# pandegroup/deepchem

Measured on AMD Instinct MI355X. Metric: molecules/sec fwd+bwd GraphConvModel, higher is better.
Workload: dtype f32; 1 GPU; Tox21-like synthetic molecules (18.2 atoms/mol, E/N 2.08), 12 binary tasks, GraphConvModel [64,64]/dense 128, BatchNorm on, fwd+bwd+Adam per step; grad_mode=full, gemm_mode=fast (split-bf16 x3 products on v_mfma_f32_32x32x16_bf16, fp32-accurate), parallelism=dp1 (molecules sharded by rank, one flat all-reduce per step)

## Files before the change

deepchem_amd/csrc/bwd_fused.hip:

```cpp
#include <atomic>
#include <type_traits>

#include "common.h"
#include "split_bf16.h"

namespace gcmi {

constexpr int kFRows = 64;
constexpr int kFMaxSeg = 16;

struct FusedTable {
  int32_t n_seg;
  int32_t seg_begin[kFMaxSeg];
  int32_t seg_end[kFMaxSeg];
  int32_t tile_start[kFMaxSeg + 1];
  int64_t w_off[2][kFMaxSeg];
  int64_t db_off[kFMaxSeg];
};

struct FusedArgs {
  const float* dy;
  int32_t lddy;
  const float* x;
  int32_t ldx;
  const float* coef;
  const int32_t* membership;
  const float* g2;
  int32_t ldg2;
  const int32_t* arg;
  const float* in[2];
  int32_t ldin[2];
  int32_t k_in;
  const float* w;
  float* dw;
  float* db;
  float* dout[2];
  int32_t lddout[2];
  double* psums;
  unsigned long long* diag;
};

template <int NG, int KT, int NOPS, bool TRANS, bool RD, bool DGRAD, bool HB = false, bool GB = false, bool IB = HB>
__global__ void __launch_bounds__(DGRAD ? 512 : 256) __attribute__((amdgpu_waves_per_eu(2)))
fused_bwd_kernel(FusedTable st, int n_tiles, FusedArgs a, int rev) {
  static_assert(!GB || HB, "bf16 gradient streams come with bf16 activations");
  static_assert(IB || !HB, "bf16 activations include the block's inputs");
  static_assert(IB == HB || !DGRAD, "In alone as bf16: the weight-gradient-only form");
  constexpr int NT = DGRAD ? 512 : 256;
  constexpr int NJ = NG / 32;
  constexpr int KP = KT * 32;
  constexpr int GP = NG + 4;
  constexpr int IP = KP + 4;
  constexpr int WP = NG + 8;
  constexpr size_t kWBytes = !DGRAD ? 0 : sizeof(unsigned short) * (size_t)NOPS * 3 * KP * WP;
  constexpr int QPR = NG / 4;
  constexpr int RPP = NT / QPR;
  constexpr int GPASS = kFRows / RPP;
  constexpr int IQ = KP / 4;
  constexpr int IPASS = kFRows * IQ / NT;
  constexpr int STEPS = kFRows / 16;
  constexpr bool INTERLEAVE = !RD;
  constexpr int OT = NOPS * KT;
  constexpr int TPW = OT / 2;
  constexpr int OP = OT * 32 + 8;
  constexpr int OQ = OT * 8;
  constexpr int OPASS = DGRAD ? kFRows * OQ / NT : 1;
  static_assert(NOPS * NJ == 4, "four weight-gradient waves: one (operand, column group) each");
  static_assert(!DGRAD || (OT % 2 == 0), "input-gradient tiles split over two waves per row block");
  static_assert(kFRows * IQ % NT == 0, "In tile loads divide evenly");
  extern __shared__ __attribute__((aligned(16))) unsigned char lds_raw[];
  float* Gs = reinterpret_cast<float*>(lds_raw);
  float* Ins = Gs + kFRows * GP;
  unsigned short* Wimg = reinterpret_cast<unsigned short*>(Ins + NOPS * kFRows * IP);
  float* Outs = reinterpret_cast<float*>(reinterpret_cast<unsigned char*>(Wimg) + kWBytes);
  __shared__ int t_begin_s[kFMaxSeg], t_end_s[kFMaxSeg], t_tile_s[kFMaxSeg + 1];
  __shared__ long long t_w_s[2][kFMaxSeg], t_db_s[kFMaxSeg];
  __shared__ __attribute__((aligned(16))) float coef_s[3 * NG];
  __shared__ double stat_s[2][DGRAD ? KP : 1];

  const int tid = threadIdx.x;
  const int wave = __builtin_amdgcn_readfirstlane(tid >> 6);
  const int lane = tid & 63;
  const int half = lane >> 5;
  const int l31 = lane & 31;
  const bool is_dgrad = DGRAD && wave < 4;
  const int wq = wave & 3;
  const int wo = wq / NJ, wj = wq % NJ;
  const int rb = wq & 1, cg = wq >> 1;

  if (tid <= kFMaxSeg) {
    t_tile_s[tid] = pick_n(st.tile_start, tid);
    if (tid < kFMaxSeg) {
      t_begin_s[tid] = pick_n(st.seg_begin, tid);
      t_end_s[tid] = pick_n(st.seg_end, tid);
      t_w_s[0][tid] = pick_n(st.w_off[0], tid);
      t_w_s[1][tid] = pick_n(st.w_off[1], tid);
      t_db_s[tid] = pick_n(st.db_off, tid);
    }
  }
  const int n_seg = st.n_seg;

  const int b = rev ? (int)gridDim.x - 1 - (int)blockIdx.x : (int)blockIdx.x;
  const int t_begin = (int)((int64_t)b * n_tiles / gridDim.x);
  const int t_end = (int)((int64_t)(b + 1) * n_tiles / gridDim.x);
  const int my_tiles = t_end - t_begin;
  auto tile_at = [&](int i) { return rev ? t_end - 1 - i : t_begin + i; };

  const int gq = tid % QPR;
  const int gr = tid / QPR;
  for (int c = tid; c < 3 * NG; c += NT) coef_s[c] = a.coef != nullptr ? a.coef[c] : (c < NG ? 1.f : 0.f);
  if constexpr (DGRAD)
    for (int c = tid; c < 2 * KP; c += NT) stat_s[c / KP][c % KP] = 0.0;

  __syncthreads();

  struct Cursor { int seg, t0, t1, r0, r1; } cur;
  auto cur_load = [&]() {
    cur.t0 = __builtin_amdgcn_readfirstlane(t_tile_s[cur.seg]);
    cur.t1 = __builtin_amdgcn_readfirstlane(t_tile_s[cur.seg + 1]);
    cur.r0 = __builtin_amdgcn_readfirstlane(t_begin_s[cur.seg]);
    cur.r1 = __builtin_amdgcn_readfirstlane(t_end_s[cur.seg]);
  };
  {
    const int first = tile_at(0);
    int sg = 0;
    for (int k = 1; k < n_seg; ++k) sg += first >= t_tile_s[k] ? 1 : 0;
    cur.seg = __builtin_amdgcn_readfirstlane(sg);
    cur_load();
  }
  auto tile_info = [&](int tile, int& seg, int& row0, int& valid) {
    while (tile >= cur.t1) { ++cur.seg; cur_load(); }
    while (tile < cur.t0) { --cur.seg; cur_load(); }
    seg = cur.seg;
    row0 = cur.r0 + (tile - cur.t0) * kFRows;
    const int left = cur.r1 - row0;
    valid = left < kFRows ? left : kFRows;
  };

  using ActV = typename std::conditional<HB, uint2, float4>::type;
  auto load_act = [](const float* base, unsigned elem) -> ActV {
    if constexpr (HB) return *reinterpret_cast<const uint2*>(reinterpret_cast<const bf16_t*>(base) + elem);
    else return *reinterpret_cast<const float4*>(base + elem);
  };
  auto act4 = [](const ActV& v) -> float4 {
    if constexpr (HB) return widen4(v);
    else return v;
  };
  using InV = typename std::conditional<IB, uint2, float4>::type;
  auto load_in = [](const float* base, unsigned elem) -> InV {
    if constexpr (IB) return *reinterpret_cast<const uint2*>(reinterpret_cast<const bf16_t*>(base) + elem);
    else return *reinterpret_cast<const float4*>(base + elem);
  };
  auto in4 = [](const InV& v) -> float4 {
    if constexpr (IB) return widen4(v);
    else return v;
  };
  using DyV = typename std::conditional<GB && !RD, uint2, float4>::type;
  DyV pdy[GPASS];
  float4 pgm[RD ? GPASS : 1];
  ActV px[GPASS];
  InV pin[NOPS][IPASS];
  int4 parg[RD ? GPASS : 1];
  int mem1[RD ? GPASS : 1];
  auto clampr = [](int r, int valid) { return r < valid ? r : valid - 1; };
  auto load_mem = [&](int row0, int valid, int (&mem)[RD ? GPASS : 1]) {
    if constexpr (RD) {
#pragma unroll
      for (int p = 0; p < GPASS; ++p) mem[p] = a.membership[(unsigned)(row0 + clampr(gr + p * RPP, valid))];
    }
  };
  auto load_src = [&](int row0, int valid) {
#pragma unroll
    for (int p = 0; p < GPASS; ++p) {
      const unsigned r = (unsigned)(row0 + clampr(gr + p * RPP, valid));
      px[p] = load_act(a.x, r * (unsigned)a.ldx + 4u * gq);
      if constexpr (RD) {
        const unsigned m = (unsigned)mem1[p];
        pdy[p] = *reinterpret_cast<const float4*>(a.g2 + (m * (unsigned)a.ldg2 + 4u * gq));
        pgm[p] = *reinterpret_cast<const float4*>(a.g2 + (m * (unsigned)a.ldg2 + NG + 4u * gq));
        parg[p] = *reinterpret_cast<const int4*>(a.arg + (m * (unsigned)NG + 4u * gq));
      } else {
        if constexpr (GB) pdy[p] = *reinterpret_cast<const uint2*>(reinterpret_cast<const bf16_t*>(a.dy) + (r * (unsigned)a.lddy + 4u * gq));
        else pdy[p] = *reinterpret_cast<const float4*>(a.dy + (r * (unsigned)a.lddy + 4u * gq));
      }
    }
#pragma unroll
    for (int o = 0; o < NOPS; ++o) {
#pragma unroll
      for (int p = 0; p < IPASS; ++p) {
        const int slot = tid + p * NT;
        const int r = slot / IQ, q = slot - r * IQ;
        const int ld = a.ldin[o];
        const int qc = 4 * q + 4 <= ld ? 4 * q : 0;
        pin[o][p] = load_in(a.in[o], (unsigned)(row0 + clampr(r, valid)) * (unsigned)ld + qc);
      }
    }
  };

  constexpr int NACC = (DGRAD && TPW > KT) ? TPW : KT;
  f32x16 accs[NACC];
#pragma unroll
  for (int t = 0; t < NACC; ++t)
#pragma unroll
    for (int i = 0; i < 16; ++i) accs[t][i] = 0.f;
  float bsum = 0.f;
  auto flush_w = [&](int seg) {
    const int64_t woff = t_w_s[NOPS == 2 ? wo : 0][seg];
    if (woff >= 0) {
      int64_t woff_lane = woff + (TRANS ? (int64_t)(wj * 32 + 4 * half) * a.k_in + l31
                                        : (int64_t)(4 * half) * NG + wj * 32 + l31);
      asm volatile("" : "+v"(woff_lane));
      float* wp = a.dw + woff_lane;
#pragma unroll
      for (int t = 0; t < KT; ++t) {
#pragma unroll
        for (int reg = 0; reg < 16; ++reg) {
          const int r8 = (reg & 3) + 8 * (reg >> 2);
          if constexpr (TRANS) {
            if (t * 32 + l31 < a.k_in) atomicAdd(wp + (int64_t)r8 * a.k_in + t * 32, accs[t][reg]);
          } else {
            if (t * 32 + r8 + 4 * half < a.k_in) atomicAdd(wp + (t * 32 + r8) * NG, accs[t][reg]);
          }
        }
      }
    }
#pragma unroll
    for (int t = 0; t < KT; ++t)
#pragma unroll
      for (int i = 0; i < 16; ++i) accs[t][i] = 0.f;
    if (wo == 0) {
      const int64_t boff = t_db_s[seg];
      const float s = bsum + __shfl_xor(bsum, 32);
      if (half == 0 && a.db != nullptr && boff >= 0) atomicAdd(a.db + boff + wj * 32 + l31, s);
    }
    bsum = 0.f;
  };

  static_assert(!DGRAD || NT % IQ == 0, "a thread keeps its column piece over the passes");
  float ps1[4] = {0.f, 0.f, 0.f, 0.f}, ps2[4] = {0.f, 0.f, 0.f, 0.f};
  auto flush_psums = [&]() {
    if constexpr (DGRAD) {
      const int q = tid % IQ;
      if (4 * q < a.k_in) {
#pragma unroll
        for (int i = 0; i < 4; ++i) {
          atomicAdd(&stat_s[0][4 * q + i], (double)ps1[i]);
          atomicAdd(&stat_s[1][4 * q + i], (double)ps2[i]);
          ps1[i] = ps2[i] = 0.f;
        }
      }
    }
  };
  auto store_out = [&](int prow0, int pvalid, int pseg) {
    if constexpr (DGRAD) {
      static_assert(OQ == NOPS * IQ, "one input-gradient row piece per In row piece");
      const float deg = (float)pseg;
#pragma unroll
      for (int o = 0; o < NOPS; ++o) {
        float* dst = o == 1 ? a.dout[1] : a.dout[0];
        const int ldd = o == 1 ? a.lddout[1] : a.lddout[0];
#pragma unroll
        for (int p = 0; p < IPASS; ++p) {
          const int slot = tid + p * NT;
          const int r = slot / IQ, q = slot - r * IQ;
          if (r < pvalid && 4 * q < a.k_in) {
            float4 v = *reinterpret_cast<const float4*>(Outs + r * OP + o * KP + 4 * q);
            if constexpr (GB) {
              const uint2 h = narrow4(v.x, v.y, v.z, v.w);
              *reinterpret_cast<uint2*>(reinterpret_cast<bf16_t*>(dst) + ((unsigned)(prow0 + r) * (unsigned)ldd + 4u * q)) = h;
              v = widen4(h);
            } else {
              *reinterpret_cast<float4*>(dst + ((unsigned)(prow0 + r) * (unsigned)ldd + 4u * q)) = v;
            }
            if (a.psums != nullptr) {
              const float4 in = *reinterpret_cast<const float4*>(Ins + (o * kFRows + r) * IP + 4 * q);
              const float wgt = (NOPS == 2 && o == 0) ? deg : 1.f;
              ps1[0] = fmaf(wgt, v.x, ps1[0]); ps1[1] = fmaf(wgt, v.y, ps1[1]);
              ps1[2] = fmaf(wgt, v.z, ps1[2]); ps1[3] = fmaf(wgt, v.w, ps1[3]);
              ps2[0] = fmaf(v.x, in.x, ps2[0]); ps2[1] = fmaf(v.y, in.y, ps2[1]);
              ps2[2] = fmaf(v.z, in.z, ps2[2]); ps2[3] = fmaf(v.w, in.w, ps2[3]);
            }
          }
        }
      }
    }
  };

  int seg, row0, valid;
  tile_info(tile_at(0), seg, row0, valid);
  int nseg = seg, nrow0 = row0, nvalid = valid;
  if (my_tiles > 1) tile_info(tile_at(1), nseg, nrow0, nvalid);
  load_mem(row0, valid, mem1);
  load_src(row0, valid);
  load_mem(nrow0, nvalid, mem1);
  int cur_seg = -1;
  int prow0 = row0, pvalid = 0, pseg = 0;

  const bool stamp = a.diag != nullptr && blockIdx.x == 0 && lane == 0 && (wave == 0 || wave == NT / 64 - 1);
  unsigned long long d_a = 0, d_w1 = 0, d_b = 0, d_w2 = 0, t0 = 0, t1 = 0;
  for (int i = 0; i < my_tiles; ++i) {
    if (stamp) t0 = wall_clock64();
    if (seg != cur_seg) {
      if (cur_seg >= 0 && !is_dgrad) flush_w(cur_seg);
      cur_seg = seg;
      if constexpr (DGRAD) {
        constexpr int NE = NOPS * KP * NG;
        for (int e = tid; e < NE; e += NT) {
          int o, ko, c;
          if constexpr (TRANS) {
            o = 0;
            c = e / KP;
            ko = e - c * KP;
          } else {
            o = e / (KP * NG);
            const int r = e - o * (KP * NG);
            ko = r / NG;
            c = r - ko * NG;
          }
          const int64_t woff = t_w_s[NOPS == 2 ? (o & 1) : 0][seg];
          float v = 0.f;
          if (woff >= 0 && ko < a.k_in)
            v = TRANS ? a.w[woff + (int64_t)c * a.k_in + ko] : a.w[woff + (int64_t)ko * NG + c];
          unsigned p1, p2, p3;
          split3(v, p1, p2, p3);
          unsigned short* dst = Wimg + ((size_t)(o * 3) * KP + ko) * WP + c;
          dst[0] = (unsigned short)(p1 >> 16);
          dst[(size_t)KP * WP] = (unsigned short)(p2 >> 16);
          dst[(size_t)2 * KP * WP] = (unsigned short)(p3 >> 16);
        }
      }
    }

    if (i > 0) {
      store_out(prow0, pvalid, pseg);
      if (a.psums != nullptr && (i & 7) == 0) flush_psums();
    }
#pragma unroll
    for (int p = 0; p < GPASS; ++p) {
      const int r = gr + p * RPP;
      float4 dy4;
      if constexpr (GB && !RD) dy4 = widen4(pdy[p]);
      else dy4 = pdy[p];
      float dyv[4] = {dy4.x, dy4.y, dy4.z, dy4.w};
      const float4 x4 = act4(px[p]);
      const float xv[4] = {x4.x, x4.y, x4.z, x4.w};
      if constexpr (RD) {
        const int rg = row0 + r;
        const float gm[4] = {pgm[p].x, pgm[p].y, pgm[p].z, pgm[p].w};
        const int av[4] = {parg[p].x, parg[p].y, parg[p].z, parg[p].w};
#pragma unroll
        for (int q = 0; q < 4; ++q) dyv[q] = dyv[q] + (av[q] == rg ? gm[q] : 0.f);
      }
      const float4 cA4 = *reinterpret_cast<const float4*>(coef_s + 4 * gq);
      const float4 cB4 = *reinterpret_cast<const float4*>(coef_s + NG + 4 * gq);
      const float4 cC4 = *reinterpret_cast<const float4*>(coef_s + 2 * NG + 4 * gq);
      const float cA[4] = {cA4.x, cA4.y, cA4.z, cA4.w}, cB[4] = {cB4.x, cB4.y, cB4.z, cB4.w};
      const float cC[4] = {cC4.x, cC4.y, cC4.z, cC4.w};
      float o[4];
#pragma unroll
      for (int q = 0; q < 4; ++q) {
        const float v = fmaf(cA[q], dyv[q], fmaf(cB[q], xv[q], cC[q]));
        o[q] = (r < valid && xv[q] > 0.f) ? v : 0.f;
      }
      *reinterpret_cast<float4*>(Gs + r * GP + 4 * gq) = make_float4(o[0], o[1], o[2], o[3]);
    }
#pragma unroll
    for (int o = 0; o < NOPS; ++o) {
#pragma unroll
      for (int p = 0; p < IPASS; ++p) {
        const int slot = tid + p * NT;
        const int r = slot / IQ, q = slot - r * IQ;
        const int tail = a.k_in - 4 * q;
        float4 v = in4(pin[o][p]);
        const bool ok = r < valid;
        v.x = (ok && tail > 0) ? v.x : 0.f;
        v.y = (ok && tail > 1) ? v.y : 0.f;
        v.z = (ok && tail > 2) ? v.z : 0.f;
        v.w = (ok && tail > 3) ? v.w : 0.f;
        *reinterpret_cast<float4*>(Ins + (o * kFRows + r) * IP + 4 * q) = v;
      }
    }
    if (stamp) { t1 = wall_clock64(); d_a += t1 - t0; }
    __syncthreads();
    if (stamp) { t0 = wall_clock64(); d_w1 += t0 - t1; }

    int n2seg = nseg, n2row0 = nrow0, n2valid = nvalid;
    if (i + 2 < my_tiles) tile_info(tile_at(i + 2), n2seg, n2row0, n2valid);
    load_src(nrow0, nvalid);
    load_mem(n2row0, n2valid, mem1);
    if (is_dgrad) {
      if constexpr (DGRAD) {
#pragma unroll
        for (int t = 0; t < TPW; ++t)
#pragma unroll
          for (int k = 0; k < 16; ++k) accs[t][k] = 0.f;
        bool on[TPW];
#pragma unroll
        for (int t = 0; t < TPW; ++t) {
          const int ot = cg * TPW + t;
          on[t] = t_w_s[NOPS == 2 ? ((ot / KT) & 1) : 0][seg] >= 0;
        }
        constexpr int NKS = NG / 16, NU = NKS * TPW;
        float4 glo, ghi;
        u32x4 wv[2][3];
        auto read_g = [&](int ks) {
          const float* grow = Gs + (rb * 32 + l31) * GP + ks * 16 + 8 * half;
          glo = *reinterpret_cast<const float4*>(grow);
          ghi = *reinterpret_cast<const float4*>(grow + 4);
        };
        auto read_w = [&](int u) {
          const int ks = u / TPW, t = u - ks * TPW;
          const int ot = cg * TPW + t;
          const int o = ot / KT, kt = ot - o * KT;
          const unsigned short* wrow = Wimg + ((size_t)(o * 3) * KP + kt * 32 + l31) * WP + ks * 16 + 8 * half;
          wv[u & 1][0] = *reinterpret_cast<const u32x4*>(wrow);
          wv[u & 1][1] = *reinterpret_cast<const u32x4*>(wrow + (size_t)KP * WP);
          if constexpr (!HB) wv[u & 1][2] = *reinterpret_cast<const u32x4*>(wrow + (size_t)2 * KP * WP);
        };
        read_g(0);
        read_w(0);
        Frag3 fg;
#pragma unroll
        for (int u = 0; u < NU; ++u) {
          const int ks = u / TPW, t = u - ks * TPW;
          if (t == 0) {
            const float v[8] = {glo.x, glo.y, glo.z, glo.w, ghi.x, ghi.y, ghi.z, ghi.w};
            fg = split_frag(v);
          }
          if (u + 1 < NU) {
            read_w(u + 1);
            if (t == TPW - 1) read_g(ks + 1);
          }
          if (on[t]) {
            const u32x4 w1 = wv[u & 1][0], w2 = wv[u & 1][1];
            if constexpr (!HB) {
              const u32x4 w3 = wv[u & 1][2];
              accs[t] = __builtin_amdgcn_mfma_f32_32x32x16_bf16(as_bf16x8(fg.p[2]), as_bf16x8(w1), accs[t], 0, 0, 0);
              accs[t] = __builtin_amdgcn_mfma_f32_32x32x16_bf16(as_bf16x8(fg.p[0]), as_bf16x8(w3), accs[t], 0, 0, 0);
              accs[t] = __builtin_amdgcn_mfma_f32_32x32x16_bf16(as_bf16x8(fg.p[1]), as_bf16x8(w2), accs[t], 0, 0, 0);
            }
            accs[t] = __builtin_amdgcn_mfma_f32_32x32x16_bf16(as_bf16x8(fg.p[1]), as_bf16x8(w1), accs[t], 0, 0, 0);
            accs[t] = __builtin_amdgcn_mfma_f32_32x32x16_bf16(as_bf16x8(fg.p[0]), as_bf16x8(w2), accs[t], 0, 0, 0);
            accs[t] = __builtin_amdgcn_mfma_f32_32x32x16_bf16(as_bf16x8(fg.p[0]), as_bf16x8(w1), accs[t], 0, 0, 0);
          }
          __builtin_amdgcn_sched_barrier(0);
        }
#pragma unroll
        for (int t = 0; t < TPW; ++t) {
          float* orow = Outs + (rb * 32 + 4 * half) * OP + (cg * TPW + t) * 32 + l31;
#pragma unroll
          for (int reg = 0; reg < 16; ++reg) orow[((reg & 3) + 8 * (reg >> 2)) * OP] = accs[t][reg];
        }
      }
    } else {
      const bool on = t_w_s[NOPS == 2 ? wo : 0][seg] >= 0;
      const float* irow = Ins + (NOPS == 2 ? wo : 0) * kFRows * IP;
      constexpr int FPS = 1 + KT, NF = STEPS * FPS;
      if constexpr (INTERLEAVE) {
      float raw[8];
      auto read_frag = [&](int f) {
        const int st_ = f / FPS, w_ = f - st_ * FPS;
        const float* src = w_ == 0 ? Gs + (16 * st_ + 8 * half) * GP + wj * 32 + l31
                                   : irow + (16 * st_ + 8 * half) * IP + (w_ - 1) * 32 + l31;
        const int pitch = w_ == 0 ? GP : IP;
#pragma unroll
        for (int u = 0; u < 8; ++u) raw[u] = src[u * pitch];
      };
      read_frag(0);
      Frag3 fg, cur, nxt;
      {
        if (wo == 0) {
#pragma unroll
          for (int u = 0; u < 8; ++u) bsum += raw[u];
        }
        nxt = split_frag(raw);
        if (NF > 1) read_frag(1);
      }
#pragma unroll
      for (int f = 0; f < NF; ++f) {
        const int w_ = f % FPS;
        cur = nxt;
        if (w_ == 0) fg = cur;
        const bool more = f + 1 < NF;
        if (more && (f + 1) % FPS == 0 && wo == 0) {
#pragma unroll
          for (int u = 0; u < 8; ++u) bsum += raw[u];
        }
        unsigned q[3][4];
        const bool next_is_g = (f + 1) % FPS == 0;
        auto pair_split = [&](int i) {
          if (!more) return;
          if (IB && !next_is_g) {
            q[0][i] = pack_exact_bf16x2(raw[2 * i], raw[2 * i + 1]);
            q[1][i] = q[2][i] = 0u;
          } else {
            split3_pair(raw[2 * i], raw[2 * i + 1], q[0][i], q[1][i], q[2][i]);
          }
        };
        if (IB && w_ != 0 && on) {
          const int t = w_ - 1;
          const Frag3& L = TRANS ? fg : cur;
          const Frag3& R = TRANS ? cur : fg;
          if constexpr (!HB) {
            accs[t] = __builtin_amdgcn_mfma_f32_32x32x16_bf16(as_bf16x8(TRANS ? L.p[2] : L.p[0]),
                                                              as_bf16x8(TRANS ? R.p[0] : R.p[2]), accs[t], 0, 0, 0);
            __builtin_amdgcn_sched_barrier(0);
          }
          pair_split(0);
          pair_split(1);
          __builtin_amdgcn_sched_barrier(0);
          accs[t] = __builtin_amdgcn_mfma_f32_32x32x16_bf16(as_bf16x8(TRANS ? L.p[1] : L.p[0]),
                                                            as_bf16x8(TRANS ? R.p[0] : R.p[1]), accs[t], 0, 0, 0);
          __builtin_amdgcn_sched_barrier(0);
          pair_split(2);
          pair_split(3);
          __builtin_amdgcn_sched_barrier(0);
          if (more && f + 2 < NF) read_frag(f + 2);
          __builtin_amdgcn_sched_barrier(0);
          accs[t] = __builtin_amdgcn_mfma_f32_32x32x16_bf16(as_bf16x8(L.p[0]), as_bf16x8(R.p[0]), accs[t], 0, 0, 0);
        } else if (w_ != 0 && on) {
          const int t = w_ - 1;
          const Frag3& L = TRANS ? fg : cur;
          const Frag3& R = TRANS ? cur : fg;
          accs[t] = __builtin_amdgcn_mfma_f32_32x32x16_bf16(as_bf16x8(L.p[2]), as_bf16x8(R.p[0]), accs[t], 0, 0, 0);
          __builtin_amdgcn_sched_barrier(0);
          pair_split(0);
          __builtin_amdgcn_sched_barrier(0);
          accs[t] = __builtin_amdgcn_mfma_f32_32x32x16_bf16(as_bf16x8(L.p[0]), as_bf16x8(R.p[2]), accs[t], 0, 0, 0);
          __builtin_amdgcn_sched_barrier(0);
          pair_split(1);
          __builtin_amdgcn_sched_barrier(0);
          accs[t] = __builtin_amdgcn_mfma_f32_32x32x16_bf16(as_bf16x8(L.p[1]), as_bf16x8(R.p[1]), accs[t], 0, 0, 0);
          __builtin_amdgcn_sched_barrier(0);
          pair_split(2);
          __builtin_amdgcn_sched_barrier(0);
          accs[t] = __builtin_amdgcn_mfma_f32_32x32x16_bf16(as_bf16x8(L.p[1]), as_bf16x8(R.p[0]), accs[t], 0, 0, 0);
          __builtin_amdgcn_sched_barrier(0);
          pair_split(3);
          __builtin_amdgcn_sched_barrier(0);
          accs[t] = __builtin_amdgcn_mfma_f32_32x32x16_bf16(as_bf16x8(L.p[0]), as_bf16x8(R.p[1]), accs[t], 0, 0, 0);
          __builtin_amdgcn_sched_barrier(0);
          if (more && f + 2 < NF) read_frag(f + 2);
          __builtin_amdgcn_sched_barrier(0);
          accs[t] = __builtin_amdgcn_mfma_f32_32x32x16_bf16(as_bf16x8(L.p[0]), as_bf16x8(R.p[0]), accs[t], 0, 0, 0);
        } else {
#pragma unroll
          for (int i = 0; i < 4; ++i) pair_split(i);
          if (more && f + 2 < NF) read_frag(f + 2);
        }
        if (more) {
#pragma unroll
          for (int pc = 0; pc < 3; ++pc) {
            nxt.p[pc].x = q[pc][0]; nxt.p[pc].y = q[pc][1]; nxt.p[pc].z = q[pc][2]; nxt.p[pc].w = q[pc][3];
          }
        }
        __builtin_amdgcn_sched_barrier(0);
      }
      } else {
      float raw[2][8];
      auto read_frag = [&](int f) {
        const int st_ = f / FPS, w_ = f - st_ * FPS;
        const float* src = w_ == 0 ? Gs + (16 * st_ + 8 * half) * GP + wj * 32 + l31
                                   : irow + (16 * st_ + 8 * half) * IP + (w_ - 1) * 32 + l31;
        const int pitch = w_ == 0 ? GP : IP;
#pragma unroll
        for (int u = 0; u < 8; ++u) raw[f & 1][u] = src[u * pitch];
      };
      read_frag(0);
      Frag3 fg;
#pragma unroll
      for (int f = 0; f < NF; ++f) {
        const int w_ = f % FPS;
        if (f + 1 < NF) read_frag(f + 1);
        if (w_ == 0) {
          if (wo == 0) {
#pragma unroll
            for (int u = 0; u < 8; ++u) bsum += raw[f & 1][u];
          }
          fg = split_frag(raw[f & 1]);
        } else if (on) {
          const int t = w_ - 1;
          if constexpr (HB) {
            u32x4 fi;
            fi.x = pack_exact_bf16x2(raw[f & 1][0], raw[f & 1][1]); fi.y = pack_exact_bf16x2(raw[f & 1][2], raw[f & 1][3]);
            fi.z = pack_exact_bf16x2(raw[f & 1][4], raw[f & 1][5]); fi.w = pack_exact_bf16x2(raw[f & 1][6], raw[f & 1][7]);
#pragma unroll
            for (int pc = 1; pc >= 0; --pc)
              accs[t] = TRANS ? __builtin_amdgcn_mfma_f32_32x32x16_bf16(as_bf16x8(fg.p[pc]), as_bf16x8(fi), accs[t], 0, 0, 0)
                              : __builtin_amdgcn_mfma_f32_32x32x16_bf16(as_bf16x8(fi), as_bf16x8(fg.p[pc]), accs[t], 0, 0, 0);
            __builtin_amdgcn_sched_barrier(0);
            continue;
          }
          const Frag3 fa = split_frag(raw[f & 1]);
          const Frag3& L = TRANS ? fg : fa;
          const Frag3& R = TRANS ? fa : fg;
          accs[t] = __builtin_amdgcn_mfma_f32_32x32x16_bf16(as_bf16x8(L.p[2]), as_bf16x8(R.p[0]), accs[t], 0, 0, 0);
          accs[t] = __builtin_amdgcn_mfma_f32_32x32x16_bf16(as_bf16x8(L.p[0]), as_bf16x8(R.p[2]), accs[t], 0, 0, 0);
          accs[t] = __builtin_amdgcn_mfma_f32_32x32x16_bf16(as_bf16x8(L.p[1]), as_bf16x8(R.p[1]), accs[t], 0, 0, 0);
          accs[t] = __builtin_amdgcn_mfma_f32_32x32x16_bf16(as_bf16x8(L.p[1]), as_bf16x8(R.p[0]), accs[t], 0, 0, 0);
          accs[t] = __builtin_amdgcn_mfma_f32_32x32x16_bf16(as_bf16x8(L.p[0]), as_bf16x8(R.p[1]), accs[t], 0, 0, 0);
          accs[t] = __builtin_amdgcn_mfma_f32_32x32x16_bf16(as_bf16x8(L.p[0]), as_bf16x8(R.p[0]), accs[t], 0, 0, 0);
        }
        __builtin_amdgcn_sched_barrier(0);
      }
      }
    }
    if (stamp) { t1 = wall_clock64(); d_b += t1 - t0; }
    __syncthreads();
    if (stamp) { t0 = wall_clock64(); d_w2 += t0 - t1; }
    prow0 = row0; pvalid = valid; pseg = seg;
    seg = nseg; row0 = nrow0; valid = nvalid;
    nseg = n2seg; nrow0 = n2row0; nvalid = n2valid;
  }
  store_out(prow0, pvalid, pseg);
  if (!is_dgrad) flush_w(cur_seg);
  if constexpr (DGRAD) {
    if (a.psums != nullptr) {
      flush_psums();
      __syncthreads();
      for (int c = tid; c < 2 * KP; c += NT) {
        const int which = c / KP, col = c - which * KP;
        if (col < a.k_in)
          atomicAdd(a.psums + (size_t)2 * a.k_in * (1 + (blockIdx.x % kBnReplicas)) + (size_t)which * a.k_in + col,
                    stat_s[which][col]);
      }
    }
  }
  if (stamp) {
    unsigned long long* d = a.diag + (wave == 0 ? 0 : 5);
    d[0] = d_a; d[1] = d_w1; d[2] = d_b; d[3] = d_w2; d[4] = (unsigned long long)my_tiles;
  }
}

static bool fused_bwd_on() {
  static const int env = getenv("GCMI_FUSED_BWD") ? atoi(getenv("GCMI_FUSED_BWD")) : 1;
  return env != 0;
}

static std::atomic<int> g_fused_bwd{1};
static std::atomic<int> g_fused_launches{0};
int fused_bwd_launches() { return g_fused_launches.load(std::memory_order_relaxed); }
void set_fused_bwd(int on) { g_fused_bwd.store(on ? 1 : 0, std::memory_order_relaxed); }
int get_fused_bwd() { return g_fused_bwd.load(std::memory_order_relaxed); }
bool fused_bwd_enabled() { return fused_bwd_on() && get_fused_bwd() != 0 && !gemm_exact_mode(); }

template <int NG, int KT, int NOPS, bool TRANS, bool RD, bool DGRAD, bool HB = false, bool GB = false, bool IB = HB>
static int launch_fused(const FusedTable& st, int n_tiles, const FusedArgs& a, hipStream_t sm) {
  constexpr int KP = KT * 32;
  size_t shmem = sizeof(float) * kFRows * (NG + 4) + sizeof(float) * (size_t)NOPS * kFRows * (KP + 4);
  if (DGRAD)
    shmem += sizeof(unsigned short) * (size_t)NOPS * 3 * KP * (NG + 8) + sizeof(float) * kFRows * (NOPS * KT * 32 + 8);
  auto kern = fused_bwd_kernel<NG, KT, NOPS, TRANS, RD, DGRAD, HB, GB, IB>;
  static LdsLimit lim;
  if (!raise_lds_limit(lim, reinterpret_cast<const void*>(kern), shmem)) return GCMI_ERR_UNSUPPORTED;
  const int per_cu = DGRAD ? 1 : 2;
  const int grid = std::min(n_tiles, 256 * per_cu);
  static const bool diag_on = getenv("GCMI_FUSED_DIAG") && atoi(getenv("GCMI_FUSED_DIAG")) != 0;
  static unsigned long long* d_diag = nullptr;
  FusedArgs aa = a;
  if (diag_on) {
    if (!d_diag && hipMalloc(&d_diag, 10 * sizeof(unsigned long long)) != hipSuccess) d_diag = nullptr;
    if (d_diag) (void)hipMemsetAsync(d_diag, 0, 10 * sizeof(unsigned long long), sm);
    aa.diag = d_diag;
  }
  hipLaunchKernelGGL(kern, dim3(grid), dim3(DGRAD ? 512 : 256), shmem, sm, st, n_tiles, aa, next_sweep_direction());
  GCMI_CHECK_LAUNCH("fused_bwd");
  if (diag_on && d_diag) {
    unsigned long long h[10];
    if (hipStreamSynchronize(sm) == hipSuccess && hipMemcpy(h, d_diag, sizeof(h), hipMemcpyDeviceToHost) == hipSuccess)
      fprintf(stderr, "fused_bwd<%d,%d,%d> tiles %llu | first wave: G phase %.2f us, wait %.2f, products %.2f, wait %.2f "
                      "| last wave: %.2f %.2f %.2f %.2f (per tile)\n", NG, KT, (int)DGRAD, h[4],
              h[0] * 0.01 / h[4], h[1] * 0.01 / h[4], h[2] * 0.01 / h[4], h[3] * 0.01 / h[4], h[5] * 0.01 / h[4],
              h[6] * 0.01 / h[4], h[7] * 0.01 / h[4], h[8] * 0.01 / h[4]);
  }
  g_fused_launches.fetch_add(1, std::memory_order_relaxed);
  return GCMI_OK;
}

static int make_table(int32_t n_seg, const int32_t* seg_begin, const int32_t* seg_end, const int64_t* w0_off,
                      const int64_t* w1_off, const int64_t* db_off, FusedTable* st) {
  memset(st, 0, sizeof(*st));
  st->n_seg = n_seg;
  int64_t tiles = 0;
  for (int s = 0; s < kFMaxSeg; ++s) {
    st->tile_start[s] = (int32_t)tiles;
    st->w_off[0][s] = st->w_off[1][s] = st->db_off[s] = -1;
    if (s < n_seg) {
      st->seg_begin[s] = seg_begin[s];
      st->seg_end[s] = seg_end[s];
      st->w_off[0][s] = w0_off ? w0_off[s] : -1;
      st->w_off[1][s] = w1_off ? w1_off[s] : -1;
      st->db_off[s] = db_off ? db_off[s] : -1;
      tiles += (seg_end[s] - seg_begin[s] + kFRows - 1) / kFRows;
    }
  }
  st->tile_start[kFMaxSeg] = (int32_t)tiles;
  return (int)tiles;
}

int fused_conv_bwd(int32_t n_seg, const int32_t* seg_begin, const int32_t* seg_end, const int64_t* w_rel,
                   const int64_t* w_self, const int64_t* b_off, const float* d_dy, int64_t lddy, const float* d_gc,
                   int64_t ldgc, const float* d_coef, int32_t width, const float* d_s, int64_t lds, const float* d_x,
                   int64_t ldx, int32_t k_in, const float* d_w, float* d_dw, float* d_dbsum, float* d_ds_out,
                   int64_t ldds, float* d_dxs_out, int64_t lddxs, double* d_psums, hipStream_t sm, int32_t act_bf16,
                   int32_t in_bf16) {
  if (!fused_bwd_enabled() || n_seg > kFMaxSeg || width != 64) return GCMI_ERR_UNSUPPORTED;
  if (in_bf16 && (act_bf16 || d_ds_out != nullptr || k_in <= 64 || k_in > 96)) return GCMI_ERR_UNSUPPORTED;
  {
    int64_t rows = 0;
    for (int sgi = 0; sgi < n_seg; ++sgi) rows = std::max<int64_t>(rows, seg_end[sgi]);
    const int64_t ldmax = std::max(std::max(lddy, ldgc), std::max(std::max(lds, ldx), std::max(ldds, lddxs)));
    if (rows * ldmax >= (int64_t)1 << 30) return GCMI_ERR_UNSUPPORTED;
  }
  if (!aligned16(d_dy) || lddy % 4 || !aligned16(d_gc) || ldgc % 4) return GCMI_ERR_UNSUPPORTED;
  if (d_coef && !aligned16(d_coef)) return GCMI_ERR_UNSUPPORTED;
  if ((act_bf16 || in_bf16) && (!aligned16(d_s) || lds % 4 || !aligned16(d_x) || ldx % 4)) return GCMI_ERR_UNSUPPORTED;
  const bool dgrad = d_ds_out != nullptr;
  FusedTable st;
  const int tiles = make_table(n_seg, seg_begin, seg_end, w_rel, w_self, b_off, &st);
  if (tiles == 0) return GCMI_OK;
  FusedArgs a;
  memset(&a, 0, sizeof(a));
  a.dy = d_dy; a.lddy = (int32_t)lddy; a.x = d_gc; a.ldx = (int32_t)ldgc; a.coef = d_coef;
  a.in[0] = d_s; a.ldin[0] = (int32_t)lds; a.in[1] = d_x; a.ldin[1] = (int32_t)ldx; a.k_in = k_in;
  a.w = d_w; a.dw = d_dw; a.db = d_dbsum;
  a.dout[0] = d_ds_out; a.lddout[0] = (int32_t)ldds; a.dout[1] = d_dxs_out; a.lddout[1] = (int32_t)lddxs;
  a.psums = dgrad ? d_psums : nullptr;
  if (dgrad) {
    if (k_in % 4 || ldds % 4 || lddxs % 4 || !aligned16(d_ds_out) || !aligned16(d_dxs_out)) return GCMI_ERR_UNSUPPORTED;
    if (k_in > 32 && k_in <= 64)
      return act_bf16 == 2 ? launch_fused<64, 2, 2, false, false, true, true, true>(st, tiles, a, sm)
             : act_bf16    ? launch_fused<64, 2, 2, false, false, true, true>(st, tiles, a, sm)
                           : launch_fused<64, 2, 2, false, false, true>(st, tiles, a, sm);
    return GCMI_ERR_UNSUPPORTED;
  }
  if (k_in > 32 && k_in <= 64)
    return act_bf16 == 2 ? launch_fused<64, 2, 2, false, false, false, true, true>(st, tiles, a, sm)
           : act_bf16    ? launch_fused<64, 2, 2, false, false, false, true>(st, tiles, a, sm)
                         : launch_fused<64, 2, 2, false, false, false>(st, tiles, a, sm);
  if (in_bf16) return launch_fused<64, 3, 2, false, false, false, false, false, true>(st, tiles, a, sm);
  if (k_in > 64 && k_in <= 96)
    return act_bf16 == 2 ? launch_fused<64, 3, 2, false, false, false, true, true>(st, tiles, a, sm)
           : act_bf16    ? launch_fused<64, 3, 2, false, false, false, true>(st, tiles, a, sm)
                         : launch_fused<64, 3, 2, false, false, false>(st, tiles, a, sm);
  return GCMI_ERR_UNSUPPORTED;
}

int fused_dense_bwd(int64_t n_rows, const int32_t* d_membership, const float* d_g2, int64_t ldg2,
                    const int32_t* d_arg, const float* d_dense, int64_t ldd, const float* d_coef, int32_t width,
                    const float* d_p, int64_t ldp, int32_t k_in, const float* d_w, float* d_dw, float* d_db,
                    float* d_dp, int64_t lddp, double* d_psums, hipStream_t sm, int32_t act_bf16) {
  if (!fused_bwd_enabled() || width != 128 || k_in <= 32 || k_in > 64 || d_coef == nullptr) return GCMI_ERR_UNSUPPORTED;
  if (!aligned16(d_g2) || ldg2 % 4 || !aligned16(d_arg) || !aligned16(d_dense) || ldd % 4 || !aligned16(d_coef))
    return GCMI_ERR_UNSUPPORTED;
  if (n_rows <= 0 || n_rows > INT32_MAX || k_in % 4 || lddp % 4 || !aligned16(d_dp)) return GCMI_ERR_UNSUPPORTED;
  if (n_rows * std::max<int64_t>(std::max(ldd, ldg2), std::max(ldp, lddp)) >= (int64_t)1 << 30) return GCMI_ERR_UNSUPPORTED;
  const int32_t zero = 0, nn = (int32_t)n_rows;
  const int64_t off0 = 0;
  FusedTable st;
  const int tiles = make_table(1, &zero, &nn, &off0, nullptr, &off0, &st);
  FusedArgs a;
  memset(&a, 0, sizeof(a));
  a.x = d_dense; a.ldx = (int32_t)ldd; a.coef = d_coef;
  a.membership = d_membership; a.g2 = d_g2; a.ldg2 = (int32_t)ldg2; a.arg = d_arg;
  a.in[0] = d_p; a.ldin[0] = (int32_t)ldp; a.k_in = k_in;
  a.w = d_w; a.dw = d_dw; a.db = d_db;
  a.dout[0] = d_dp; a.lddout[0] = (int32_t)lddp;
  a.psums = d_psums;
  if (act_bf16) {
    if (!aligned16(d_p) || ldp % 4) return GCMI_ERR_UNSUPPORTED;
    if (act_bf16 == 2) return launch_fused<128, 2, 1, true, true, true, true, true>(st, tiles, a, sm);
    return launch_fused<128, 2, 1, true, true, true, true>(st, tiles, a, sm);
  }
  return launch_fused<128, 2, 1, true, true, true>(st, tiles, a, sm);
}

}
```

Measured before the change: 21.91 million molecules/s.

## Split dense-layer backward operands to bf16 triples once when staging into LDS

For the fp32 dense-layer fused backward, the gradient tile and the input tile are split into three bf16 parts when written to shared memory, using swizzled layouts. Previously they were stored as fp32 and split again inside each MFMA fragment read. The weight-gradient waves now read fragments with ds_read_tr16 transposed loads, and the input-gradient waves read the pre-split G image directly. The bias gradient is reduced in LDS per segment before one global atomic, and the changed layout needs a different LDS footprint. The intent is to remove repeated split arithmetic and fp32 fragment gathers in the inner MFMA loops, at the cost of rebuilding the input values from three parts for the BatchNorm partial sums and adding an extra block barrier at each bias flush.

```diff
diff --git a/deepchem_amd/csrc/bwd_fused.hip b/deepchem_amd/csrc/bwd_fused.hip
--- a/deepchem_amd/csrc/bwd_fused.hip
+++ b/deepchem_amd/csrc/bwd_fused.hip
@@ -8,6 +8,11 @@
 
 constexpr int kFRows = 64;
 constexpr int kFMaxSeg = 16;
+
+__device__ __forceinline__ uint2 lds_read_tr16(const unsigned char* p) {
+  typedef short s16x4 __attribute__((ext_vector_type(4)));
+  return __builtin_bit_cast(uint2, __builtin_amdgcn_ds_read_tr16_b64_v4i16((__attribute__((address_space(3))) s16x4*)p));
+}
 
 struct FusedTable {
   int32_t n_seg;
@@ -40,9 +45,12 @@
   unsigned long long* diag;
 };
 
-template <int NG, int KT, int NOPS, bool TRANS, bool RD, bool DGRAD, bool HB = false, bool GB = false, bool IB = HB>
+template <int NG, int KT, int NOPS, bool TRANS, bool RD, bool DGRAD, bool HB = false, bool GB = false, bool IB = HB,
+          bool SO = false>
 __global__ void __launch_bounds__(DGRAD ? 512 : 256) __attribute__((amdgpu_waves_per_eu(2)))
 fused_bwd_kernel(FusedTable st, int n_tiles, FusedArgs a, int rev) {
+  static_assert(!SO || (NG == 128 && KT == 2 && NOPS == 1 && TRANS && RD && DGRAD && !HB && !GB && !IB),
+                "split-once: the fp32 dense-layer form");
   static_assert(!GB || HB, "bf16 gradient streams come with bf16 activations");
   static_assert(IB || !HB, "bf16 activations include the block's inputs");
   static_assert(IB == HB || !DGRAD, "In alone as bf16: the weight-gradient-only form");
@@ -71,8 +79,16 @@
   extern __shared__ __attribute__((aligned(16))) unsigned char lds_raw[];
   float* Gs = reinterpret_cast<float*>(lds_raw);
   float* Ins = Gs + kFRows * GP;
-  unsigned short* Wimg = reinterpret_cast<unsigned short*>(Ins + NOPS * kFRows * IP);
+  constexpr int kGImg = kFRows * NG * 2;
+  constexpr int kIImg = kFRows * KP * 2;
+  unsigned char* Gimg = lds_raw;
+  unsigned char* Iimg = lds_raw + 3 * kGImg;
+  unsigned short* Wimg = SO ? reinterpret_cast<unsigned short*>(Iimg + 3 * kIImg)
+                            : reinterpret_cast<unsigned short*>(Ins + NOPS * kFRows * IP);
   float* Outs = reinterpret_cast<float*>(reinterpret_cast<unsigned char*>(Wimg) + kWBytes);
+  float* db_s = Outs + kFRows * OP;
+  auto g_swz = [](int row) { return ((row & 3) << 2) | ((row >> 2) & 3); };
+  auto i_swz = [](int row) { return ((row >> 1) & 1) << 2; };
   __shared__ int t_begin_s[kFMaxSeg], t_end_s[kFMaxSeg], t_tile_s[kFMaxSeg + 1];
   __shared__ long long t_w_s[2][kFMaxSeg], t_db_s[kFMaxSeg];
   __shared__ __attribute__((aligned(16))) float coef_s[3 * NG];
@@ -111,6 +127,8 @@
   for (int c = tid; c < 3 * NG; c += NT) coef_s[c] = a.coef != nullptr ? a.coef[c] : (c < NG ? 1.f : 0.f);
   if constexpr (DGRAD)
     for (int c = tid; c < 2 * KP; c += NT) stat_s[c / KP][c % KP] = 0.0;
+  if constexpr (SO)
+    for (int c = tid; c < NG; c += NT) db_s[c] = 0.f;
 
   __syncthreads();
 
@@ -228,12 +246,31 @@
     for (int t = 0; t < KT; ++t)
 #pragma unroll
       for (int i = 0; i < 16; ++i) accs[t][i] = 0.f;
-    if (wo == 0) {
-      const int64_t boff = t_db_s[seg];
-      const float s = bsum + __shfl_xor(bsum, 32);
-      if (half == 0 && a.db != nullptr && boff >= 0) atomicAdd(a.db + boff + wj * 32 + l31, s);
-    }
-    bsum = 0.f;
+    if constexpr (!SO) {
+      if (wo == 0) {
+        const int64_t boff = t_db_s[seg];
+        const float s = bsum + __shfl_xor(bsum, 32);
+        if (half == 0 && a.db != nullptr && boff >= 0) atomicAdd(a.db + boff + wj * 32 + l31, s);
+      }
+      bsum = 0.f;
+    }
+  };
+  float bs4[4] = {0.f, 0.f, 0.f, 0.f};
+  auto flush_db = [&](int seg) {
+    if constexpr (SO) {
+#pragma unroll
+      for (int q = 0; q < 4; ++q) {
+        const float s = bs4[q] + __shfl_xor(bs4[q], 32);
+        if (half == 0) atomicAdd(&db_s[4 * gq + q], s);
+        bs4[q] = 0.f;
+      }
+      __syncthreads();
+      if (tid < NG) {
+        const int64_t boff = t_db_s[seg];
+        if (a.db != nullptr && boff >= 0) atomicAdd(a.db + boff + tid, db_s[tid]);
+        db_s[tid] = 0.f;
+      }
+    }
   };
 
   static_assert(!DGRAD || NT % IQ == 0, "a thread keeps its column piece over the passes");
@@ -273,7 +310,16 @@
               *reinterpret_cast<float4*>(dst + ((unsigned)(prow0 + r) * (unsigned)ldd + 4u * q)) = v;
             }
             if (a.psums != nullptr) {
-              const float4 in = *reinterpret_cast<const float4*>(Ins + (o * kFRows + r) * IP + 4 * q);
+              float4 in;
+              if constexpr (SO) {
+                const unsigned char* src = Iimg + 128 * r + 16 * ((q >> 1) ^ i_swz(r)) + 8 * (q & 1);
+                const float4 i1 = widen4(*reinterpret_cast<const uint2*>(src));
+                const float4 i2 = widen4(*reinterpret_cast<const uint2*>(src + kIImg));
+                const float4 i3 = widen4(*reinterpret_cast<const uint2*>(src + 2 * kIImg));
+                in = make_float4((i1.x + i2.x) + i3.x, (i1.y + i2.y) + i3.y, (i1.z + i2.z) + i3.z, (i1.w + i2.w) + i3.w);
+              } else {
+                in = *reinterpret_cast<const float4*>(Ins + (o * kFRows + r) * IP + 4 * q);
+              }
               const float wgt = (NOPS == 2 && o == 0) ? deg : 1.f;
               ps1[0] = fmaf(wgt, v.x, ps1[0]); ps1[1] = fmaf(wgt, v.y, ps1[1]);
               ps1[2] = fmaf(wgt, v.z, ps1[2]); ps1[3] = fmaf(wgt, v.w, ps1[3]);
@@ -302,6 +348,7 @@
     if (stamp) t0 = wall_clock64();
     if (seg != cur_seg) {
       if (cur_seg >= 0 && !is_dgrad) flush_w(cur_seg);
+      if (cur_seg >= 0) flush_db(cur_seg);
       cur_seg = seg;
       if constexpr (DGRAD) {
         constexpr int NE = NOPS * KP * NG;
@@ -362,7 +409,19 @@
         const float v = fmaf(cA[q], dyv[q], fmaf(cB[q], xv[q], cC[q]));
         o[q] = (r < valid && xv[q] > 0.f) ? v : 0.f;
       }
-      *reinterpret_cast<float4*>(Gs + r * GP + 4 * gq) = make_float4(o[0], o[1], o[2], o[3]);
+      if constexpr (SO) {
+        unsigned a1, a2, a3, b1, b2, b3;
+        split3_pair(o[0], o[1], a1, a2, a3);
+        split3_pair(o[2], o[3], b1, b2, b3);
+        unsigned char* dst = Gimg + 256 * r + 16 * ((gq >> 1) ^ g_swz(r)) + 8 * (gq & 1);
+        *reinterpret_cast<uint2*>(dst) = make_uint2(a1, b1);
+        *reinterpret_cast<uint2*>(dst + kGImg) = make_uint2(a2, b2);
+        *reinterpret_cast<uint2*>(dst + 2 * kGImg) = make_uint2(a3, b3);
+#pragma unroll
+        for (int q = 0; q < 4; ++q) bs4[q] += o[q];
+      } else {
+        *reinterpret_cast<float4*>(Gs + r * GP + 4 * gq) = make_float4(o[0], o[1], o[2], o[3]);
+      }
     }
 #pragma unroll
     for (int o = 0; o < NOPS; ++o) {
@@ -377,7 +436,17 @@
         v.y = (ok && tail > 1) ? v.y : 0.f;
         v.z = (ok && tail > 2) ? v.z : 0.f;
         v.w = (ok && tail > 3) ? v.w : 0.f;
-        *reinterpret_cast<float4*>(Ins + (o * kFRows + r) * IP + 4 * q) = v;
+        if constexpr (SO) {
+          unsigned a1, a2, a3, b1, b2, b3;
+          split3_pair(v.x, v.y, a1, a2, a3);
+          split3_pair(v.z, v.w, b1, b2, b3);
+          unsigned char* dst = Iimg + 128 * r + 16 * ((q >> 1) ^ i_swz(r)) + 8 * (q & 1);
+          *reinterpret_cast<uint2*>(dst) = make_uint2(a1, b1);
+          *reinterpret_cast<uint2*>(dst + kIImg) = make_uint2(a2, b2);
+          *reinterpret_cast<uint2*>(dst + 2 * kIImg) = make_uint2(a3, b3);
+        } else {
+          *reinterpret_cast<float4*>(Ins + (o * kFRows + r) * IP + 4 * q) = v;
+        }
       }
     }
     if (stamp) { t1 = wall_clock64(); d_a += t1 - t0; }
@@ -389,7 +458,47 @@
     load_src(nrow0, nvalid);
     load_mem(n2row0, n2valid, mem1);
     if (is_dgrad) {
-      if constexpr (DGRAD) {
+      if constexpr (SO) {
+        static_assert(TPW == 1, "one output tile per input-gradient wave");
+#pragma unroll
+        for (int k = 0; k < 16; ++k) accs[0][k] = 0.f;
+        const bool on = t_w_s[0][seg] >= 0;
+        constexpr int NKS = NG / 16;
+        int ln = lane;
+        asm volatile("" : "+v"(ln));
+        const int half = ln >> 5, l31 = ln & 31;
+        const int grow = rb * 32 + l31;
+        const unsigned char* gbase = Gimg + 256 * grow;
+        const int gsw = g_swz(grow);
+        const unsigned short* wbase = Wimg + ((size_t)cg * 32 + l31) * WP + 8 * half;
+        u32x4 gv[2][3], wv[2][3];
+        auto read_k = [&](int ks) {
+          const unsigned char* gp = gbase + 16 * ((2 * ks + half) ^ gsw);
+#pragma unroll
+          for (int pc = 0; pc < 3; ++pc) {
+            gv[ks & 1][pc] = *reinterpret_cast<const u32x4*>(gp + pc * kGImg);
+            wv[ks & 1][pc] = *reinterpret_cast<const u32x4*>(wbase + (size_t)pc * KP * WP + ks * 16);
+          }
+        };
+        read_k(0);
+#pragma unroll
+        for (int ks = 0; ks < NKS; ++ks) {
+          if (ks + 1 < NKS) read_k(ks + 1);
+          if (on) {
+            const u32x4 *g = gv[ks & 1], *w = wv[ks & 1];
+            accs[0] = __builtin_amdgcn_mfma_f32_32x32x16_bf16(as_bf16x8(g[2]), as_bf16x8(w[0]), accs[0], 0, 0, 0);
+            accs[0] = __builtin_amdgcn_mfma_f32_32x32x16_bf16(as_bf16x8(g[0]), as_bf16x8(w[2]), accs[0], 0, 0, 0);
+            accs[0] = __builtin_amdgcn_mfma_f32_32x32x16_bf16(as_bf16x8(g[1]), as_bf16x8(w[1]), accs[0], 0, 0, 0);
+            accs[0] = __builtin_amdgcn_mfma_f32_32x32x16_bf16(as_bf16x8(g[1]), as_bf16x8(w[0]), accs[0], 0, 0, 0);
+            accs[0] = __builtin_amdgcn_mfma_f32_32x32x16_bf16(as_bf16x8(g[0]), as_bf16x8(w[1]), accs[0], 0, 0, 0);
+            accs[0] = __builtin_amdgcn_mfma_f32_32x32x16_bf16(as_bf16x8(g[0]), as_bf16x8(w[0]), accs[0], 0, 0, 0);
+          }
+          __builtin_amdgcn_sched_barrier(0);
+        }
+        float* orow = Outs + (rb * 32 + 4 * half) * OP + cg * 32 + l31;
+#pragma unroll
+        for (int reg = 0; reg < 16; ++reg) orow[((reg & 3) + 8 * (reg >> 2)) * OP] = accs[0][reg];
+      } else if constexpr (DGRAD) {
 #pragma unroll
         for (int t = 0; t < TPW; ++t)
 #pragma unroll
@@ -456,7 +565,52 @@
       const bool on = t_w_s[NOPS == 2 ? wo : 0][seg] >= 0;
       const float* irow = Ins + (NOPS == 2 ? wo : 0) * kFRows * IP;
       constexpr int FPS = 1 + KT, NF = STEPS * FPS;
-      if constexpr (INTERLEAVE) {
+      if constexpr (SO) {
+      int ln = lane;
+      asm volatile("" : "+v"(ln));
+      const int half = ln >> 5;
+      const int tq = (ln >> 2) & 3, tp = ln & 3, cb = (ln >> 4) & 1;
+      const unsigned char *gsrc[2], *isrc[2][KT];
+#pragma unroll
+      for (int s = 0; s < 2; ++s) {
+        const int rl = 8 * half + 4 * s + tq;
+        gsrc[s] = Gimg + 256 * rl + 16 * ((4 * wj + 2 * cb + (tp >> 1)) ^ g_swz(rl)) + 8 * (tp & 1);
+#pragma unroll
+        for (int t = 0; t < KT; ++t)
+          isrc[s][t] = Iimg + 128 * rl + 16 * ((4 * t + 2 * cb + (tp >> 1)) ^ i_swz(rl)) + 8 * (tp & 1);
+      }
+      Frag3 fb[3], fg;
+      auto read_frag = [&](int f) {
+        const int st_ = f / FPS, w_ = f - st_ * FPS;
+#pragma unroll
+        for (int pc = 0; pc < 3; ++pc) {
+          const unsigned char* s0 = w_ == 0 ? gsrc[0] + st_ * 16 * 256 + pc * kGImg : isrc[0][w_ - 1] + st_ * 16 * 128 + pc * kIImg;
+          const unsigned char* s1 = w_ == 0 ? gsrc[1] + st_ * 16 * 256 + pc * kGImg : isrc[1][w_ - 1] + st_ * 16 * 128 + pc * kIImg;
+          const uint2 lo = lds_read_tr16(s0), hi = lds_read_tr16(s1);
+          fb[f % 3].p[pc].x = lo.x; fb[f % 3].p[pc].y = lo.y; fb[f % 3].p[pc].z = hi.x; fb[f % 3].p[pc].w = hi.y;
+        }
+      };
+      read_frag(0);
+      read_frag(1);
+#pragma unroll
+      for (int f = 0; f < NF; ++f) {
+        const int w_ = f % FPS;
+        const Frag3 cur = fb[f % 3];
+        if (f + 2 < NF) read_frag(f + 2);
+        if (w_ == 0) {
+          fg = cur;
+        } else if (on) {
+          const int t = w_ - 1;
+          accs[t] = __builtin_amdgcn_mfma_f32_32x32x16_bf16(as_bf16x8(fg.p[2]), as_bf16x8(cur.p[0]), accs[t], 0, 0, 0);
+          accs[t] = __builtin_amdgcn_mfma_f32_32x32x16_bf16(as_bf16x8(fg.p[0]), as_bf16x8(cur.p[2]), accs[t], 0, 0, 0);
+          accs[t] = __builtin_amdgcn_mfma_f32_32x32x16_bf16(as_bf16x8(fg.p[1]), as_bf16x8(cur.p[1]), accs[t], 0, 0, 0);
+          accs[t] = __builtin_amdgcn_mfma_f32_32x32x16_bf16(as_bf16x8(fg.p[1]), as_bf16x8(cur.p[0]), accs[t], 0, 0, 0);
+          accs[t] = __builtin_amdgcn_mfma_f32_32x32x16_bf16(as_bf16x8(fg.p[0]), as_bf16x8(cur.p[1]), accs[t], 0, 0, 0);
+          accs[t] = __builtin_amdgcn_mfma_f32_32x32x16_bf16(as_bf16x8(fg.p[0]), as_bf16x8(cur.p[0]), accs[t], 0, 0, 0);
+        }
+        __builtin_amdgcn_sched_barrier(0);
+      }
+      } else if constexpr (INTERLEAVE) {
       float raw[8];
       auto read_frag = [&](int f) {
         const int st_ = f / FPS, w_ = f - st_ * FPS;
@@ -614,6 +768,7 @@
   }
   store_out(prow0, pvalid, pseg);
   if (!is_dgrad) flush_w(cur_seg);
+  flush_db(cur_seg);
   if constexpr (DGRAD) {
     if (a.psums != nullptr) {
       flush_psums();
@@ -644,13 +799,17 @@
 int get_fused_bwd() { return g_fused_bwd.load(std::memory_order_relaxed); }
 bool fused_bwd_enabled() { return fused_bwd_on() && get_fused_bwd() != 0 && !gemm_exact_mode(); }
 
-template <int NG, int KT, int NOPS, bool TRANS, bool RD, bool DGRAD, bool HB = false, bool GB = false, bool IB = HB>
+template <int NG, int KT, int NOPS, bool TRANS, bool RD, bool DGRAD, bool HB = false, bool GB = false, bool IB = HB,
+          bool SO = false>
 static int launch_fused(const FusedTable& st, int n_tiles, const FusedArgs& a, hipStream_t sm) {
   constexpr int KP = KT * 32;
   size_t shmem = sizeof(float) * kFRows * (NG + 4) + sizeof(float) * (size_t)NOPS * kFRows * (KP + 4);
   if (DGRAD)
     shmem += sizeof(unsigned short) * (size_t)NOPS * 3 * KP * (NG + 8) + sizeof(float) * kFRows * (NOPS * KT * 32 + 8);
-  auto kern = fused_bwd_kernel<NG, KT, NOPS, TRANS, RD, DGRAD, HB, GB, IB>;
+  if (SO)
+    shmem += 3 * sizeof(unsigned short) * kFRows * (NG + KP) + sizeof(float) * NG
+             - (sizeof(float) * kFRows * (NG + 4) + sizeof(float) * (size_t)NOPS * kFRows * (KP + 4));
+  auto kern = fused_bwd_kernel<NG, KT, NOPS, TRANS, RD, DGRAD, HB, GB, IB, SO>;
   static LdsLimit lim;
   if (!raise_lds_limit(lim, reinterpret_cast<const void*>(kern), shmem)) return GCMI_ERR_UNSUPPORTED;
   const int per_cu = DGRAD ? 1 : 2;
@@ -772,7 +931,7 @@
     if (act_bf16 == 2) return launch_fused<128, 2, 1, true, true, true, true, true>(st, tiles, a, sm);
     return launch_fused<128, 2, 1, true, true, true, true>(st, tiles, a, sm);
   }
-  return launch_fused<128, 2, 1, true, true, true>(st, tiles, a, sm);
+  return launch_fused<128, 2, 1, true, true, true, false, false, false, true>(st, tiles, a, sm);
 }
 
 }
```

After: 21.89 million molecules/s. About the same (-0.1%).
